# facebookresearch/robust_cvd

Hardware: AMD Instinct MI355X
Metric: GN/LM iterations/sec (and ms/iter) on 300-frame 384x224 video, 1/2/4/8 GPU (higher is better)
Workload: dtype f64

## Files before the change

### include/cvd_hip_debug.h

```cpp
#ifndef CVD_HIP_DEBUG_H
#define CVD_HIP_DEBUG_H

#include "cvd_hip.h"

#ifdef __cplusplus
extern "C" {
#endif

typedef struct cvd_debug_options {
  uint64_t struct_size;
  int32_t force_iterations;
  int32_t force_sharded_path;
  int32_t pcg_lockstep;
  int32_t stall_fused_tail_once;
} cvd_debug_options;
void cvd_debug_options_default(cvd_debug_options* o);
int32_t cvd_set_debug_options(cvd_handle* h, const cvd_debug_options* o);

int32_t cvd_set_generic_kernels(cvd_handle* h, int32_t enabled);

int32_t cvd_comm_init_local_group(cvd_handle* h, int32_t rank, int32_t world, uint64_t group_key);
int32_t cvd_comm_init_phantom(cvd_handle* h, int32_t rank, int32_t world);

int32_t cvd_block_inverse_debug(cvd_handle* h, int32_t num_blocks, int32_t block_size, const double* a, int32_t variant,
                                float* inverse, int32_t* failed);

int32_t cvd_epipolar_debug(cvd_handle* h, int32_t num_pairs, const int64_t* offsets, const float* loc, double pixel_scale,
                           double threshold_px, int32_t iterations, uint64_t seed, uint8_t* is_static_out,
                           double* fundamental_out, int32_t* best_out, int32_t* counts_out, double* hypotheses_out);
int32_t cvd_flow_masks_debug(cvd_handle* h, int32_t num_frames, int32_t height, int32_t width, int32_t channels,
                             const float* color, int32_t num_pairs, const int32_t* pair_frames, const float* flow_ab,
                             const float* flow_ba, float flow_thresh, float color_thresh, uint8_t* mask_ab, uint8_t* mask_ba,
                             int32_t* kept, float* errors, double* kernel_ms, int32_t pixels_per_thread);
int32_t cvd_dense_inverse_debug(cvd_handle* h, int32_t n, const double* a, double* inverse, int32_t* failed);
int32_t cvd_coarse_debug(cvd_handle* h, int32_t* num_unknowns, double* a_c, double* a_c_inverse, int32_t* failed);
int32_t cvd_temporal_debug(cvd_handle* h, int32_t* dims6, double* a_t, double* a_t_inverse, double* lam, int32_t* failed);
int32_t cvd_product_launch_debug(cvd_handle* h, int32_t* out6);

#ifdef __cplusplus
}
#endif
#endif
```

### robust_cvd_amd/api.py

```python
import ctypes as C
import os
import sys

from . import build as _build
from .binding import Binding
from .ctypes_types import OptParams, SolveSummary, XformDesc

_lib = None
_variant = None


class SolverOptions(C.Structure):
    _fields_ = [
        ("struct_size", C.c_uint64),
        ("pcg_relative_tolerance", C.c_double),
        ("pcg_max_iterations", C.c_int32),
        ("verbose", C.c_int32),
        ("coarse_level", C.c_int32),
        ("robust_loss", C.c_int32),
        ("dense_matrix_free", C.c_int32),
        ("block_inverse_variant", C.c_int32),
        ("coarse_dense_max_unknowns", C.c_int32),
        ("coarse_rebuild_excess", C.c_int32),
        ("coarse_update_budget", C.c_int64),
# ... 316 lines not shown
        if not os.path.exists(path):
            raise ImportError(
                f"{path} is missing: build it with `python -c 'import __graft_entry__ as g; g.build()'` "
                "(hipcc --offload-arch=gfx950). robust_cvd_amd has no CPU fallback.")
        lib = C.CDLL(path)
        lib.cvd_create.restype = C.c_void_p
        lib.cvd_create.argtypes = [C.c_int32]
        lib.cvd_last_error.restype = C.c_char_p
        lib.cvd_last_error.argtypes = [C.c_void_p]
        lib.cvd_num_active_constraints.restype = C.c_int64
        lib.cvd_abi_revision.restype = C.c_int32
        if lib.cvd_abi_revision() != ABI_REVISION:
            raise ImportError(f"{path} was built with ABI revision {lib.cvd_abi_revision()}, this binding is written against "
                              f"{ABI_REVISION} (include/cvd_hip.h: CVD_ABI_REVISION): rebuild the library")
        _lib = lib
        _variant = variant
    return _lib


def loaded_variant():
    return _variant


EXPORTED_SYMBOLS = [
    "cvd_create", "cvd_destroy", "cvd_last_error", "cvd_abi_sizes", "cvd_opt_params_default",
    "cvd_solver_options_default", "cvd_set_solver_options", "cvd_debug_options_default", "cvd_set_debug_options", "cvd_set_generic_kernels", "cvd_comm_unique_id", "cvd_comm_init", "cvd_comm_init_local_group", "cvd_comm_init_phantom", "cvd_set_pair_graph", "cvd_set_video", "cvd_set_depth", "cvd_set_depth_all",
    "cvd_set_pair_constraints", "cvd_set_pair_flows", "cvd_dense_mode_supported", "cvd_set_triplet_constraints", "cvd_set_poses", "cvd_get_poses",
    "cvd_reset_poses", "cvd_reset_depth_xforms", "cvd_reset_spatial_xforms", "cvd_grid_xform_split",
    "cvd_get_xform_desc", "cvd_num_xform_params", "cvd_get_xform_params", "cvd_set_xform_params",
    "cvd_get_pose_params", "cvd_set_pose_params", "cvd_block_size", "cvd_normalize_depth", "cvd_pose_optimization",
    "cvd_pose_optimization_step", "cvd_evaluate", "cvd_sample_pair_constraints", "cvd_get_sampled_constraints", "cvd_sample_triplet_constraints", "cvd_get_sampled_triplet_constraints", "cvd_set_dynamic_masks", "cvd_corner_min_eigenval", "cvd_dynamic_distance", "cvd_apply_depth_xforms", "cvd_depth_param_maps", "cvd_spatial_warp_maps", "cvd_flow_guided_filter", "cvd_bilateral_filter", "cvd_epipolar_static_flags", "cvd_compute_tracks", "cvd_get_tracks", "cvd_flow_consistency_masks", "cvd_consistency_loss", "cvd_consistency_loss_device", "cvd_scene_flow_loss", "cvd_scene_flow_loss_device", "cvd_spatial_losses", "cvd_spatial_losses_device", "cvd_param_chunk", "cvd_parameter_l1", "cvd_parameter_l1_device", "cvd_param_step", "cvd_param_step_device", "cvd_dataset_create", "cvd_dataset_clear", "cvd_dataset_set_colors", "cvd_dataset_set_flows", "cvd_dataset_set_depth_orig", "cvd_dataset_set_cameras", "cvd_dataset_set_xforms", "cvd_dataset_set_maps", "cvd_dataset_batch", "cvd_dataset_batch_device", "cvd_dataset_bad_indices", "cvd_get_summary", "cvd_num_records", "cvd_get_records",
    "cvd_get_kernel_times", "cvd_get_comm_times", "cvd_get_dense_times", "cvd_set_kernel_timing", "cvd_num_active_constraints", "cvd_coarse_debug", "cvd_temporal_debug", "cvd_path_info", "cvd_abi_revision",
    "cvd_block_inverse_debug", "cvd_dense_inverse_debug", "cvd_epipolar_debug", "cvd_flow_masks_debug",
    "cvd_product_launch_debug",
]

KERNEL_CLASSES = ["evaluate_assemble", "matvec_pairs", "matvec_finish", "cg_update", "block_inverse", "cost"]


class Solver(Binding):
    def __init__(self, device=0):
        lib = load_library()
        handle = lib.cvd_create(C.c_int32(device))
        if not handle:
            raise RuntimeError("cvd_create failed: " + (lib.cvd_last_error(None) or b"").decode())
        super().__init__(lib, "cvd_", handle)
        self._options = None
        self._debug = None

    def set_options(self, pcg_relative_tolerance=None, pcg_max_iterations=None, verbose=None,
                    coarse_level=None, robust_loss=None, **variants):
        debug = {k: variants.pop(k) for k in list(variants) if k in dict(DebugOptions._fields_) and k != "struct_size"}
        if debug:
            d = self._debug
            if d is None:
                d = DebugOptions()
                self._lib.cvd_debug_options_default(C.byref(d))
                self._debug = d
            for k, v in debug.items():
                setattr(d, k, int(v))
            self._check(self._fn("set_debug_options")(self._h, C.byref(d)))
        o = self._options
        if o is None:
            o = SolverOptions()
            self._lib.cvd_solver_options_default(C.byref(o))
            self._options = o
        if pcg_relative_tolerance is not None:
# ... 430 lines not shown
                                                    out.ctypes.data_as(C.POINTER(C.c_double)), C.byref(fl)))
        return out, fl.value

    def temporal_debug(self):
        import numpy as np
        dims = (C.c_int32 * 6)()
        self._check(self._fn("temporal_debug")(self._h, dims, None, None, None, None))
        if dims[0] == 0:
            return None
        n = dims[0]
        a = np.zeros((n, n))
        ai = np.zeros((n, n))
        lam = np.zeros(self.num_frames * self.block_size())
        fl = C.c_int32(0)
        dp = lambda x: x.ctypes.data_as(C.POINTER(C.c_double))
        self._check(self._fn("temporal_debug")(self._h, dims, dp(a), dp(ai), dp(lam), C.byref(fl)))
        return {"NT": n, "S": dims[1], "nn": dims[2], "step": dims[3], "Sx": dims[4], "Sy": dims[5], "a_t": a, "a_t_inverse": ai,
                "lam": lam, "failed": fl.value}

    def path_info(self):
        out = (C.c_int32 * 8)()
        self._check(self._fn("path_info")(self._h, out))
        form = {-1: "none", 0: "exact sparse factor", 1: "exact dense inverse", 2: "temporal pose level"}[out[1]]
        return {"pose_graph_level": form, "depth_grid_level": bool(out[2]), "fused_tail": bool(out[3]), "tail_disabled": bool(out[4]),
                "taps": out[5], "work_items": out[6], "cross_blocks": bool(out[7])}

    def product_launch_debug(self):
        out = (C.c_int32 * 6)()
        self._check(self._fn("product_launch_debug")(self._h, out))
        kind = {-1: "none", 0: "generic list", 1: "fast list", 2: "fast dense", 3: "cross blocks"}[out[3]]
        return {"threads": out[0], "spec": out[1], "kd": out[2], "kind": out[3], "kind_name": kind, "work_items": out[4],
                "num_cu": out[5]}

    def coarse_debug(self):
        import numpy as np
        n = C.c_int32(0)
        self._check(self._fn("coarse_debug")(self._h, C.byref(n), None, None, None))
        if n.value == 0:
            return None
        a = np.zeros((n.value, n.value))
        ai = np.zeros((n.value, n.value))
        fl = C.c_int32(0)
        self._check(self._fn("coarse_debug")(self._h, C.byref(n), a.ctypes.data_as(C.POINTER(C.c_double)),
                                             ai.ctypes.data_as(C.POINTER(C.c_double)), C.byref(fl)))
        return {"a_c": a, "a_c_inverse": ai, "failed": fl.value}
```

### robust_cvd_amd/csrc/cvd_api.hip

```cpp
#include "cvd_host.h"
#include "cvd_coarse.h"

namespace cvd {

static void poseOptimizationStep(cvd_handle* h, const cvd_opt_params& p, double depthDeformReg) {
  solve(h, p, depthDeformReg, PK_POSE_STEP);
  paramsToPoses(h, p);
}

static void poseOptimization(cvd_handle* h, const cvd_opt_params& p) {
  posesToParams(h);
  h->records.clear();
  int ctfRows = p.ctf_long, ctfCols = p.ctf_short;
  int dsoRows = p.dso_long, dsoCols = p.dso_short;
  if (h->aspect >= 1.f) {
    std::swap(ctfCols, ctfRows);
    std::swap(dsoCols, dsoRows);
  }
  int initGrid[3] = {1, 1, 1};
  if (h->ddesc.depth_type == CVD_DEPTH_GRID)
    for (int i = 0; i < 3; ++i) initGrid[i] = h->ddesc.grid_size[i];
  const int Nval = (h->ddesc.depth_type == CVD_DEPTH_IDENTITY) ? 0 : valueNumParams(h->ddesc.value_xform);
  size_t nDmax = static_cast<size_t>(h->nD());
  if (p.coarse_to_fine && h->ddesc.depth_type != CVD_DEPTH_IDENTITY && p.num_steps > 1)
// ... 889 lines not shown
  CVD_TRY(h, {
    auto& T = h->temporal;
    hipStream_t s = h->stream;
    const bool on = T.on && T.built;
    const int dims[6] = {on ? T.NT : 0, T.S, T.nn, T.step, T.Sx, T.Sy};
    for (int i = 0; i < 6; ++i) dims6[i] = dims[i];
    if (on) {
      const size_t n2 = static_cast<size_t>(T.NT) * T.NT;
      if (a_t) T.A.download(a_t, n2, s);
      if (a_t_inverse) T.Ainv.download(a_t_inverse, n2, s);
      if (lam) h->dLam.download(lam, static_cast<size_t>(h->F) * h->Bsz(), s);
      int fl = 0;
      T.fail.download(&fl, 1, s);
      HIP_CHECK(hipStreamSynchronize(s));
      if (failed) *failed = fl;
    }
  });
}
int32_t cvd_path_info(cvd_handle* h, int32_t* out8) {
  CVD_TRY(h, {
    out8[0] = h->coarseOn ? 1 : 0;
    out8[1] = !h->coarseOn ? -1 : (h->coarse.temporalPose ? 2 : (h->coarse.denseMode ? 1 : 0));
    out8[2] = h->temporal.on ? 1 : 0;
    out8[3] = h->lastFusedTail ? 1 : 0;
    out8[4] = h->tailDisabled ? 1 : 0;
    out8[5] = h->lastKD;
    out8[6] = static_cast<int32_t>(h->itemFa.size());
    out8[7] = h->lastCross ? 1 : 0;
  });
}
int32_t cvd_product_launch_debug(cvd_handle* h, int32_t* out6) {
  CVD_TRY(h, {
    for (int i = 0; i < 6; ++i) out6[i] = h->lastProduct[i];
  });
}
int32_t cvd_coarse_debug(cvd_handle* h, int32_t* num_unknowns, double* a_c, double* a_c_inverse, int32_t* failed) {
  CVD_TRY(h, {
    auto& C = h->coarse;
    if (!C.valid || !h->coarseOn) {
      *num_unknowns = 0;
    } else if (C.temporalPose) {
      const size_t n = static_cast<size_t>(C.ptN);
      *num_unknowns = static_cast<int32_t>(n);
      hipStream_t s = h->stream;
      int fl = 0;
      C.fail.download(&fl, 1, s);
      if (a_c) C.ptMat.download(a_c, n * n, s);
      if (a_c_inverse) C.ptInv.download(a_c_inverse, n * n, s);
      HIP_CHECK(hipStreamSynchronize(s));
      if (failed) *failed = fl;
    } else {
      const int F = h->F;
      const size_t n = static_cast<size_t>(F) * kCB;
      *num_unknowns = static_cast<int32_t>(n);
      hipStream_t s = h->stream;
      int fl = 0;
      C.fail.download(&fl, 1, s);
      if (a_c_inverse) {
        std::vector<double> save(n), unit(n, 0.0);
        C.rc.download(save.data(), n, s);
        HIP_CHECK(hipStreamSynchronize(s));
        DevBuf<double> scalTmp;
        scalTmp.ensure(S_COUNT);
        HIP_CHECK(hipMemsetAsync(scalTmp.p, 0, S_COUNT * sizeof(double), s));
        for (size_t k = 0; k < n; ++k) {
          unit[k] = 1.0;
// ... 47 lines not shown
```

### robust_cvd_amd/csrc/cvd_assembly.h

```cpp
#pragma once

#include "cvd_kernels.h"

namespace cvd {

template <int KD, int KS>
inline __global__ __launch_bounds__(256) void k_assemble(Layout L, Table T, const double* __restrict__ x,
                                                  const FrameConst* __restrict__ fc, const double* __restrict__ mask,
                                                  const float* __restrict__ median,
                                                  const unsigned char* __restrict__ inRange,
                                                  const unsigned char* __restrict__ rangeFlags,
                                                  const int* __restrict__ fpOff, const int* __restrict__ fpList,
                                                  double* __restrict__ gOut, double* __restrict__ hOut,
                                                  double* __restrict__ costFrame, double* __restrict__ focalG,
                                                  double* __restrict__ focalH, AsmPanels panels, int panelCap) {
  extern __shared__ __attribute__((aligned(16))) double sm[];
  const int B = L.B;
  double* Hs = sm;
  double* gs = Hs + panelCap;
  double* xf = gs + B;
  double* xo = xf + B;
  FrameConst* fcs = reinterpret_cast<FrameConst*>(xo + B);
  double* red = reinterpret_cast<double*>(fcs + 2);
  const int f = blockIdx.x;
// ... 210 lines not shown
inline __global__ __launch_bounds__(256) void k_shared_focal_fixup(Layout L, const double* __restrict__ focalG,
                                                            const double* __restrict__ focalH,
                                                            const double* __restrict__ mask, double* __restrict__ g,
                                                            double* __restrict__ hBlocks) {
  __shared__ double red[8];
  double a = 0.0, b = 0.0;
  for (int f = threadIdx.x; f < L.F; f += 256) { a += focalG[f]; b += focalH[f]; }
  a = waveSum(a);
  b = waveSum(b);
  if ((threadIdx.x & 63) == 0) { red[threadIdx.x >> 6] = a; red[4 + (threadIdx.x >> 6)] = b; }
  __syncthreads();
  if (threadIdx.x == 0) {
    const double m = mask[6];
    g[6] += (red[0] + red[1] + red[2] + red[3]) * m;
    hBlocks[static_cast<size_t>(6) * L.B + 6] += (red[4] + red[5] + red[6] + red[7]) * m * m;
  }
}

inline __global__ void k_extract_diag(Layout L, const double* __restrict__ hBlocks, double* __restrict__ out) {
  const size_t n = static_cast<size_t>(L.F) * L.B;
  const size_t i = static_cast<size_t>(blockIdx.x) * blockDim.x + threadIdx.x;
  if (i >= n) return;
  const size_t f = i / L.B, c = i - f * L.B;
  out[i] = hBlocks[(f * L.B + c) * L.B + c];
}


#ifdef CVD_ASM_PROFILE
__device__ unsigned long long g_asmProf[2048 * 16];
#define ASM_STAMP(slot) do { if (lane == 0) g_asmProf[(blockIdx.x & 2047) * 16 + (slot)] = wall_clock64(); } while (0)
#else
#define ASM_STAMP(slot) do {} while (0)
#endif
template <int KD, bool DENSE = false, bool STAGE = false, bool FOLD = false>
inline __global__ __launch_bounds__(kAsmThreads) void k_assemble_fast(Layout L, Table T, const double* __restrict__ x,
                                                       const FrameConst* __restrict__ fc,
                                                       const double* __restrict__ mask, const float* __restrict__ median,
                                                       const unsigned char* __restrict__ regOwner,
                                                       const unsigned char* __restrict__ rangeFlags,
                                                       AsmWork work,
                                                       double* __restrict__ gOut, double* __restrict__ hOut,
                                                       double* __restrict__ costFrame, double* __restrict__ focalG,
                                                       double* __restrict__ focalH, DenseRecords dr = DenseRecords{}) {
  extern __shared__ __attribute__((aligned(16))) double sm[];
  constexpr double eps = 1e-6;
  const int B = L.B;
  const int npk = B * (B + 1) / 2;
  double* Hs = sm;
  double* gs = Hs + npk;
  double* xf = gs + B;
  double* red = xf + B;
  double* xstage = red + 4 * 36;
  const AsmPart me = FOLD ? AsmPart{static_cast<int>(blockIdx.x), 0, 0, 0, 1, 0} : work.parts[blockIdx.x];
  const int f = me.frame;
  const int tid = threadIdx.x;
  constexpr int NT = kAsmThreads;
  const int wv = __builtin_amdgcn_readfirstlane(tid >> 6);
  const int lane = tid & 63;
  if (tid == 0) ASM_STAMP(0);
  for (int i = tid; i < npk; i += NT) Hs[i] = 0.0;
  if (tid < 48) red[tid] = 0.0;
  for (int i = tid; i < B; i += NT) {
    gs[i] = 0.0;
    xf[i] = x[static_cast<size_t>(f) * B + i];
  }
  __syncthreads();
  if (tid == 0) ASM_STAMP(1);

  double PP[28], gp[7];
  double GD[19];
#pragma unroll
  for (int i = 0; i < 19; ++i) GD[i] = 0.0;
  double cost = 0.0;
  double shG = 0.0, shH = 0.0;
#pragma unroll
  for (int i = 0; i < 28; ++i) PP[i] = 0.0;
#pragma unroll
  for (int i = 0; i < 7; ++i) gp[i] = 0.0;
  const int N = L.N;
  const double A = L.aspect;

  if constexpr (FOLD) {
    if (L.includeStatic) {
      const int G = L.nD;
      const int recN = dwRecordDoubles(G);
      const int e0 = dr.fpOff[f], e1 = dr.fpOff[f + 1];
      const int nOut = 36 + 13 * G;
      for (int o = tid; o < nOut; o += NT) {
        int off0, off1, c = -1, v = 0;
        if (o < 28) {
          int i = 0;
          while ((i + 1) * (i + 2) / 2 <= o) ++i;
          const int j = o - i * (i + 1) / 2;
          off0 = i * 16 + j;
          off1 = (7 + i) * 16 + 7 + j;
        } else if (o < 35) {
          off0 = (o - 28) * 16 + 14;
          off1 = (7 + o - 28) * 16 + 14;
        } else if (o == 35) {
          off0 = 256 + 40 * G;
          off1 = -1;
        } else {
          const int e = o - 36;
          c = e / G;
          v = e - c * G;
          if (c < 7) { off0 = 256 + c * G + v; off1 = 256 + 15 * G + (7 + c) * G + v; }
          else if (c == 7) { off0 = 256 + 14 * G + v; off1 = 256 + 29 * G + v; }
          else { off0 = 256 + 30 * G + (c - 8) * G + v; off1 = 256 + 35 * G + (c - 8) * G + v; }
        }
        double s = 0.0;
        for (int e = e0; e < e1; ++e) {
          const int code = dr.fpList[e];
          const int off = (code & 1) ? off1 : off0;
          if (off < 0) continue;
          for (int q = dr.recOff[code >> 1]; q < dr.recOff[(code >> 1) + 1]; ++q) s += dr.records[static_cast<size_t>(q) * recN + off];
        }
        if (o < 36) atomicAdd(&red[o], s);
        else if (c < 7) Hs[packedIdx(7 + v, c)] = s;
        else if (c == 7) gs[7 + v] = s;
        else {
          const int d = c - 8;
          const int v2 = v + (d == 0 ? 0 : (d == 1 ? 1 : L.gx + d - 3));
          if (v2 < G) atomicAdd(&Hs[packedIdx(7 + v2, 7 + v)], s);
        }
      }
    }
  } else
  if (L.includeStatic) {
    for (int u = me.u0 + wv; u < me.u1; u += NT / 64) {
      const int2 unit = work.units[u];
      const int code = __builtin_amdgcn_readfirstlane(unit.x);
      const int p = code >> 1;
      const int side = code & 1;
      const int o = side ? T.pairA[p] : T.pairB[p];
      const double* __restrict__ xo = x + static_cast<size_t>(o) * B;
      const FrameConst& Fa = side ? fc[o] : fc[f];
      const FrameConst& Fb = side ? fc[f] : fc[o];
      double* xw = xstage + wv * B;
      if constexpr (STAGE) {
        for (int i = lane; i < B; i += 64) xw[i] = xo[i];
        asm volatile("s_waitcnt vmcnt(0) lgkmcnt(0)" ::: "memory");
      }
      const double* xa = STAGE ? (side ? xw : xf) : (side ? xo : xf);
      const double* xb = STAGE ? (side ? xf : xw) : (side ? xf : xo);
      const double fya = Fa.fy, fxa = Fa.fy * A;
      const double fyb = Fb.fy;
      const double ifyb = 1.0 / fyb, ifxb = 1.0 / (fyb * A);
      const long long cBegin = T.pairOff[p] + __builtin_amdgcn_readfirstlane(unit.y);
      constexpr int kUnit = DENSE ? kAsmUnitDense : kAsmUnit;
      const long long cEnd = cBegin + kUnit < T.pairOff[p + 1] ? cBegin + kUnit : T.pairOff[p + 1];
      const int fsrc = side ? o : f, ftgt = side ? f : o;
      const long long cFirst = DENSE ? cBegin + static_cast<long long>(lane) * kDenseRun : cBegin + lane;
      const long long cStop = DENSE ? (cFirst + kDenseRun < cEnd ? cFirst + kDenseRun : cEnd) : cEnd;
      constexpr long long cStep = DENSE ? 1 : 64;
      RecordStream<true> rs;
      const int iFirst = static_cast<int>(cFirst - cBegin), iStop = static_cast<int>(cStop - cBegin);
      if constexpr (DENSE) rs.prime(T, cBegin, iFirst, iStop);
      for (long long c = cFirst; c < cStop; c += cStep) {
        float4 nd;
        float2 d;
        if constexpr (DENSE) {
          if (!rs.take(T, cBegin, static_cast<int>(c - cBegin), 1, iStop, T.pairOff[p], fsrc, ftgt, nd, d)) continue;
        } else {
          if (!loadConstraint<false>(T, c, T.pairOff[p], fsrc, ftgt, nd, d)) continue;
        }
        const double da = static_cast<double>(d.x), db = static_cast<double>(d.y);
        FastTaps<KD> ta, tb;
        fastGather<KD>(L, nd.x, nd.y, ta);
        fastGather<KD>(L, nd.z, nd.w, tb);
        double Da, Db;
        if (N == 0) {
// ... 234 lines not shown
#pragma unroll
        for (int i = 0; i < 19; ++i) GD[i] = waveSum(GD[i]);
        if (lane == 0) {
          for (int a = 0; a < N; ++a) {
            const int ct = 7 + a;
            for (int i = 0; i < 7; ++i) atomicAdd(&Hs[ct * (ct + 1) / 2 + i], GD[a * 7 + i]);
            atomicAdd(&gs[ct], GD[17 + a]);
          }
          atomicAdd(&Hs[packedIdx(7, 7)], GD[14]);
          if (N == 2) { atomicAdd(&Hs[packedIdx(8, 7)], GD[15]); atomicAdd(&Hs[packedIdx(8, 8)], GD[16]); }
        }
      }
    }
    if (lane == 0) {
#pragma unroll
      for (int i = 0; i < 28; ++i) atomicAdd(&red[i], PP[i]);
#pragma unroll
      for (int i = 0; i < 7; ++i) atomicAdd(&red[28 + i], gp[i]);
      atomicAdd(&red[35], cost);
    }
  }
  __syncthreads();
  if (tid < 28) {
    int i = 0;
    while ((i + 1) * (i + 2) / 2 <= tid) ++i;
    const int j = tid - i * (i + 1) / 2;
    Hs[packedIdx(i, j)] += red[tid];
  } else if (tid < 35) {
    gs[tid - 28] += red[tid];
  }
  __syncthreads();
  const double staticCost = 0.5 * red[35];
  __syncthreads();
  if (tid == 0) ASM_STAMP(13);
  if (L.intrOpt == kIntrShared) {
    shG = waveSum(shG);
    shH = waveSum(shH);
    if (lane == 0) { red[wv] = shG; red[16 + wv] = shH; }
    __syncthreads();
    if (tid == 0) {
      double sg = 0.0, sh = 0.0;
      for (int w = 0; w < NT / 64; ++w) { sg += red[w]; sh += red[16 + w]; }
      focalG[f] = sg;
      focalH[f] = sh;
      red[42] = sg;
      red[43] = sh;
      gs[6] = 0.0;
      Hs[packedIdx(6, 6)] = 0.0;
    }
    if (f != 0) {
      for (int j = tid; j < B; j += NT)
        if (j != 6) Hs[j > 6 ? packedIdx(j, 6) : packedIdx(6, j)] = 0.0;
    }
    __syncthreads();
  }

  if (tid == 0) ASM_STAMP(14);
  double regCost = 0.0;
  if (regOwner[f] && me.part == 0) {
    const int nr = numRegResiduals<KD>(L);
    for (int i = tid; i < nr; i += NT) {
      double r;
      int n;
      int cols[2 * KD + 2];
      double jac[2 * KD + 2];
      regResidual<KD>(L, f, i, xf, median[f], r, n, cols, jac);
      regCost += r * r;
      for (int a = 0; a < n; ++a) {
        atomicAdd(&gs[cols[a]], jac[a] * r);
        for (int b = 0; b <= a; ++b) {
          const int hi = cols[a] > cols[b] ? cols[a] : cols[b];
          const int lo = cols[a] > cols[b] ? cols[b] : cols[a];
          atomicAdd(&Hs[packedIdx(hi, lo)], jac[a] * jac[b]);
        }
      }
    }
  }
  if (tid == 0 && L.positionRegSqrt > 0.0 && me.part == 0) {
    double o3[3] = {0, 0, 0}, dg = 0.0, cst = 0.0;
    posRegFrame(L, rangeFlags, f, x, nullptr, o3, dg, cst);
    for (int i = 0; i < 3; ++i) {
      atomicAdd(&gs[i], o3[i]);
      atomicAdd(&Hs[packedIdx(i, i)], dg);
    }
    regCost += cst;
  }
  regCost = waveSum(regCost);
  __syncthreads();
  if (tid == 0) ASM_STAMP(15);
  if (lane == 0) red[wv] = regCost;
  __syncthreads();
// ... 55 lines not shown
```

### robust_cvd_amd/csrc/cvd_eval.hip

```cpp
#include "cvd_host.h"
#include "cvd_cost.h"
#include "cvd_assembly.h"
#include "cvd_triplets.h"
#include "cvd_dense_walk.h"

namespace cvd {

void launchFrameConsts(Ctx& c, const double* x) {
  launchFrameConsts(c.L, x, c.h->dFc.p, c.h->stream);
  HIP_CHECK(hipGetLastError());
}

void spinStream(hipStream_t s) {
  hipError_t e;
  while ((e = hipStreamQuery(s)) == hipErrorNotReady) {}
  HIP_CHECK(e);
}
void spinEvent(hipEvent_t ev) {
  hipError_t e;
  while ((e = hipEventQuery(ev)) == hipErrorNotReady) {}
  HIP_CHECK(e);
}
void readScalars(Ctx& c) {
  HIP_CHECK(hipMemcpyAsync(c.h->hScal, c.h->dScal.p, S_COUNT * sizeof(double), hipMemcpyDeviceToHost, c.h->stream));
// ... 94 lines not shown
  (void)x;
  cvd_handle* h = c.h;
  const size_t B = c.L.B, G = c.L.nD;
  h->dXBlocks.ensure(h->xFa.size() * B * B);
  const unsigned nP = static_cast<unsigned>(h->xFa.size());
  if (nP == 0) return;
  hipLaunchKernelGGL(k_dense_fold_cross, dim3(nP), dim3(256), 0, h->stream, c.L, crossPairs(h), h->dXDir.p, h->dDwRecOff.p,
                     h->dDwRecords.p, h->dXBlocks.p);
  int panelW = static_cast<int>(((kMaxLds - 4096) / 8) / G);
  panelW = std::max(1, std::min<int>(panelW, static_cast<int>(G)));
  const int nPanels = static_cast<int>((G + panelW - 1) / panelW);
  panelW = static_cast<int>((G + nPanels - 1) / nPanels);
  const size_t ldsGrid = static_cast<size_t>(panelW) * G * 8;
  allowLds((k_dense_gg<4>), ldsGrid);
  const int slot = h->tBegin(KC_DENSE_GG);
  for (int dir = 0; dir < 2; ++dir)
    hipLaunchKernelGGL((k_dense_gg<4>), dim3(nP, nPanels), dim3(kGgThreads), ldsGrid, h->stream, c.L, c.T, crossPairs(h), h->dXDir.p,
                       h->dDwGg.p, panelW, dir, h->dXBlocks.p);
  h->tEnd(slot);
  HIP_CHECK(hipGetLastError());
}

double evalFull(Ctx& c, const double* x, bool withStats, bool noReadBack) {
  cvd_handle* h = c.h;
  hipStream_t s = h->stream;
  launchFrameConsts(c, x);
  const size_t B = c.L.B;
  const int slot = h->tBegin(KC_ASSEMBLE);
  const bool fast = !h->forceGeneric && c.KS == 0 && fastLoss(c.L);
  const size_t ldsFast = (B * (B + 1) / 2 + 2 * B + 4 * 36) * 8;
  const size_t ldsRest = 3 * B * 8 + 2 * sizeof(FrameConst) + 4 * 36 * 8;
  int panelCap = 0;
  const bool fastFits = ldsFast <= kMaxLds;
  if (fast && fastFits) {
    h->dAsmScratch.ensure(static_cast<size_t>(h->nAsmSlots) * (B * (B + 1) / 2 + B + 4));
    const AsmWork work{h->dAsmParts.p, h->dAsmUnits.p, h->dAsmScratch.p, h->dAsmCount.p};
    const size_t ldsStage = ldsFast + static_cast<size_t>(kAsmThreads / 64) * B * 8;
    const bool stage = ldsStage <= kMaxLds;
#define CVD_LAUNCH_ASM(DENSEV, STAGEV)                                                                                     \
    CVD_DISPATCH_KD(c.KD, {                                                                                              \
      allowLds((k_assemble_fast<KD, DENSEV, STAGEV>), STAGEV ? ldsStage : ldsFast);                                        \
      hipLaunchKernelGGL((k_assemble_fast<KD, DENSEV, STAGEV>), dim3(h->nAsmParts), dim3(kAsmThreads), STAGEV ? ldsStage : ldsFast, s, \
                         c.L, c.T, x, h->dFc.p, h->dMask.p, h->dMedian.p, h->dRegOwner.p, h->dInRange.p, work, h->dG.p, h->dH.p,  \
                         h->dCostFrame.p, h->dFocal.p, h->dFocal.p + c.L.F);                                             \
    })
#ifndef CVD_ASM_STAGE
#define CVD_ASM_STAGE 1
#endif
    if (c.cross) {
      launchDenseWalk(c, x);
      if (c.KD == 1) {
        allowLds((k_assemble_fast<1, true, false, true>), ldsFast);
        hipLaunchKernelGGL((k_assemble_fast<1, true, false, true>), dim3(c.L.F), dim3(kAsmThreads), ldsFast, s, c.L, c.T, x, h->dFc.p,
                           h->dMask.p, h->dMedian.p, h->dRegOwner.p, h->dInRange.p, work, h->dG.p, h->dH.p, h->dCostFrame.p,
                           h->dFocal.p, h->dFocal.p + c.L.F, denseRecords(h));
      } else {
        allowLds((k_assemble_fast<4, true, false, true>), ldsFast);
        hipLaunchKernelGGL((k_assemble_fast<4, true, false, true>), dim3(c.L.F), dim3(kAsmThreads), ldsFast, s, c.L, c.T, x, h->dFc.p,
                           h->dMask.p, h->dMedian.p, h->dRegOwner.p, h->dInRange.p, work, h->dG.p, h->dH.p, h->dCostFrame.p,
                           h->dFocal.p, h->dFocal.p + c.L.F, denseRecords(h));
      }
    } else if (h->dense) { if (stage && CVD_ASM_STAGE) CVD_LAUNCH_ASM(true, true); else CVD_LAUNCH_ASM(true, false); }
    else { if (stage && CVD_ASM_STAGE) CVD_LAUNCH_ASM(false, true); else CVD_LAUNCH_ASM(false, false); }
#undef CVD_LAUNCH_ASM
  } else {
    if (h->dense && c.L.includeStatic) throw std::logic_error("dense mode: the generic assembly has no images to read (DenseListScope should have taken this solve)");
    const AsmPanels panels = makePanels(static_cast<int>(B), (kMaxLds - ldsRest) / 8, panelCap);
    const size_t lds = static_cast<size_t>(panelCap) * 8 + ldsRest;
    CVD_DISPATCH(c.KD, c.KS, {
      allowLds(k_assemble<KD, KS>, lds);
      hipLaunchKernelGGL((k_assemble<KD, KS>), dim3(c.L.F), dim3(256), lds, s, c.L, c.T, x, h->dFc.p, h->dMask.p,
                         h->dMedian.p, h->dRegOwner.p, h->dInRange.p, h->dFpOff.p, h->dFpList.p, h->dG.p, h->dH.p, h->dCostFrame.p,
                       h->dFocal.p, h->dFocal.p + c.L.F, panels, panelCap);
    });
  }
  HIP_CHECK(hipGetLastError());
  if (c.trip && c.TT.nGroups > 0) {
    int panelCapT = 0;
    const AsmPanels panelsT = makePanels(static_cast<int>(B), (kMaxLds - B * 8 - 256) / 8, panelCapT);
    const size_t ldsT = (static_cast<size_t>(panelCapT) + B) * 8;
    CVD_DISPATCH(c.KD, c.KS, {
      allowLds(k_assemble_triplets<KD, KS>, ldsT);
      hipLaunchKernelGGL((k_assemble_triplets<KD, KS>), dim3(c.L.F), dim3(256), ldsT, s, c.L, c.TT, x, h->dFc.p,
                         h->dMask.p, h->dFtOff.p, h->dFtList.p, h->dG.p, h->dH.p, h->dFocal.p, h->dFocal.p + c.L.F,
                         panelsT, panelCapT);
      hipLaunchKernelGGL((k_cost_triplets<KD, KS>), dim3(c.TT.nGroups), dim3(256), 0, s, c.L, c.TT, x, h->dFc.p,
                         h->dCostFrame.p);
    });
    HIP_CHECK(hipGetLastError());
  }
  if (c.L.intrOpt == CVD_INTR_SHARED) {
    hipLaunchKernelGGL(k_shared_focal_fixup, dim3(1), dim3(256), 0, s, c.L, h->dFocal.p, h->dFocal.p + c.L.F, h->dMask.p,
                       h->dG.p, h->dH.p);
    HIP_CHECK(hipGetLastError());
  }
  if (c.cross) launchCrossAssemble(c, x);
  h->tEnd(slot);
  if (h->dist()) {
    const int ct = h->tBegin(KC_COMM_EVAL);
    const size_t chunkH = static_cast<size_t>(h->ownChunk()) * B * B;
    commGroupStart(h);
// ... 40 lines not shown
```

### robust_cvd_amd/csrc/cvd_host.h

```cpp
#pragma once

#include <hip/hip_runtime.h>
#include <hip/hip_ext.h>
#include <rccl/rccl.h>
#include <rocblas/rocblas.h>
#include <rocsolver/rocsolver.h>

#include <algorithm>
#include <array>
#include <atomic>
#include <chrono>
#include <condition_variable>
#include <cmath>
#include <cstdarg>
#include <cstdint>
#include <cstdio>
#include <cstdlib>
#include <cstring>
#include <functional>
#include <limits>
#include <map>
#include <memory>
#include <mutex>
#include <set>
// ... 293 lines not shown
    DevBuf<unsigned char> elV;
    DevBuf<double> Cf, E, part, A, Ainv, sq, rT, t, tl, dotPart, rec;
    DevBuf<double> invPanel;
    DevBuf<unsigned int> invBarrier;
    DevBuf<TlStep> stepDev;
    hipEvent_t evIn = nullptr, evDone = nullptr;
    bool sidePending = false;
    double* sqPtr = nullptr;
  } temporal;
  hipEvent_t evRebuild[2] = {nullptr, nullptr};
  bool rebuildTimed = false;
  double coarseRebuildMs = 0.0, pcgIterMs = 0.0;
  std::vector<std::pair<int, int>> globalEdges;
  bool haveGlobalEdges = false;
  DevBuf<double> dRegJac;
  DevBuf<unsigned short> dRegCol;
  DevBuf<unsigned char> dRegCnt;
  RegCache regCache{};
  DevBuf<FrameConst> dFc;
  DevBuf<int> dFail;
  DevBuf<unsigned long long> dCount;
  double* hScal = nullptr;
  double* hStage[2] = {nullptr, nullptr};
  size_t hStageN[2] = {0, 0};
  double* hPcg = nullptr;
  hipEvent_t pcgEvent[2] = {nullptr, nullptr};

  cvd_solve_summary summary{};
  std::vector<cvd_iteration_record> records;

  bool lastFusedTail = false, lastCross = false;
  int lastKD = 0;
  int lastProduct[6] = {0, 0, 0, -1, 0, 0};
  bool tailDisabled = false;
  bool forceGeneric = false;

  int timing = 0;
  int timingStride = 1;
  long long timingCounter = 0;
  long long timingCounterKc[16] = {0};
  std::vector<std::pair<hipEvent_t, hipEvent_t>> evPool;
  std::vector<int> evClass;
  std::vector<int> evIter;
  int curPcgIter = -1;
  size_t evUsed = 0;
  double kcMs[KC_TOTAL] = {0};
  long long kcN[KC_TOTAL] = {0};

  ~cvd_handle_t() {
    for (auto& e : evPool) { (void)hipEventDestroy(e.first); (void)hipEventDestroy(e.second); }
    if (rbMain) (void)rocblas_destroy_handle(rbMain);
    if (comm) (void)ncclCommDestroy(comm);
    if (localGroup) leaveLocalGroup(*localGroup);
    if (hScal) (void)hipHostFree(hScal);
    for (auto& p : hStage) if (p) (void)hipHostFree(p);
    if (hPcg) (void)hipHostFree(hPcg);
    for (auto& e : pcgEvent) if (e) (void)hipEventDestroy(e);
    for (auto& e : evRebuild) if (e) (void)hipEventDestroy(e);
    if (temporal.evIn) (void)hipEventDestroy(temporal.evIn);
    if (temporal.evDone) (void)hipEventDestroy(temporal.evDone);
    if (evCoarseIn) (void)hipEventDestroy(evCoarseIn);
    if (evCoarseDone) (void)hipEventDestroy(evCoarseDone);
    if (evInvIn) (void)hipEventDestroy(evInvIn);
    if (evInvDone) (void)hipEventDestroy(evInvDone);
    if (stream3) (void)hipStreamDestroy(stream3);
    if (stream2) (void)hipStreamDestroy(stream2);
// ... 319 lines not shown
```

Measured before the change: 321.8.

## Add loss-specialised list-mode assembly walk for single-camera static disparity

Adds a templated SPEC variant of the fast assembly kernel, used when there is a single camera with static reprojection-disparity loss and non-shared intrinsics. The residual and Jacobian walk is specialised by robust-loss kind, with uniform hoisted rotations and fast reciprocals. The local-to-axis-angle rotation and the regulariser accumulation are moved into dedicated helpers. The aim is to cut per-constraint branching and generic overhead in Gauss-Newton assembly. It also adds a debug query reporting the chosen assembly launch and per-frame cost, and it duplicates a lot of numerics, which risks divergence from the generic path.

```diff
diff --git a/include/cvd_hip_debug.h b/include/cvd_hip_debug.h
--- a/include/cvd_hip_debug.h
+++ b/include/cvd_hip_debug.h
@@ -36,6 +36,7 @@
 int32_t cvd_coarse_debug(cvd_handle* h, int32_t* num_unknowns, double* a_c, double* a_c_inverse, int32_t* failed);
 int32_t cvd_temporal_debug(cvd_handle* h, int32_t* dims6, double* a_t, double* a_t_inverse, double* lam, int32_t* failed);
 int32_t cvd_product_launch_debug(cvd_handle* h, int32_t* out6);
+int32_t cvd_assembly_launch_debug(cvd_handle* h, int32_t* out6, double* cost_frame);
 
 #ifdef __cplusplus
 }
diff --git a/robust_cvd_amd/api.py b/robust_cvd_amd/api.py
--- a/robust_cvd_amd/api.py
+++ b/robust_cvd_amd/api.py
@@ -372,7 +372,7 @@
     "cvd_pose_optimization_step", "cvd_evaluate", "cvd_sample_pair_constraints", "cvd_get_sampled_constraints", "cvd_sample_triplet_constraints", "cvd_get_sampled_triplet_constraints", "cvd_set_dynamic_masks", "cvd_corner_min_eigenval", "cvd_dynamic_distance", "cvd_apply_depth_xforms", "cvd_depth_param_maps", "cvd_spatial_warp_maps", "cvd_flow_guided_filter", "cvd_bilateral_filter", "cvd_epipolar_static_flags", "cvd_compute_tracks", "cvd_get_tracks", "cvd_flow_consistency_masks", "cvd_consistency_loss", "cvd_consistency_loss_device", "cvd_scene_flow_loss", "cvd_scene_flow_loss_device", "cvd_spatial_losses", "cvd_spatial_losses_device", "cvd_param_chunk", "cvd_parameter_l1", "cvd_parameter_l1_device", "cvd_param_step", "cvd_param_step_device", "cvd_dataset_create", "cvd_dataset_clear", "cvd_dataset_set_colors", "cvd_dataset_set_flows", "cvd_dataset_set_depth_orig", "cvd_dataset_set_cameras", "cvd_dataset_set_xforms", "cvd_dataset_set_maps", "cvd_dataset_batch", "cvd_dataset_batch_device", "cvd_dataset_bad_indices", "cvd_get_summary", "cvd_num_records", "cvd_get_records",
     "cvd_get_kernel_times", "cvd_get_comm_times", "cvd_get_dense_times", "cvd_set_kernel_timing", "cvd_num_active_constraints", "cvd_coarse_debug", "cvd_temporal_debug", "cvd_path_info", "cvd_abi_revision",
     "cvd_block_inverse_debug", "cvd_dense_inverse_debug", "cvd_epipolar_debug", "cvd_flow_masks_debug",
-    "cvd_product_launch_debug",
+    "cvd_product_launch_debug", "cvd_assembly_launch_debug",
 ]
 
 KERNEL_CLASSES = ["evaluate_assemble", "matvec_pairs", "matvec_finish", "cg_update", "block_inverse", "cost"]
@@ -869,6 +869,15 @@
         return {"threads": out[0], "spec": out[1], "kd": out[2], "kind": out[3], "kind_name": kind, "work_items": out[4],
                 "num_cu": out[5]}
 
+    def assembly_launch_debug(self):
+        import numpy as np
+        out = (C.c_int32 * 6)()
+        cost = np.zeros(self.num_frames, dtype=np.float64)
+        self._check(self._fn("assembly_launch_debug")(self._h, out, cost.ctypes.data_as(C.POINTER(C.c_double))))
+        kind = {-1: "none", 0: "generic", 1: "fast list", 2: "fast dense", 3: "dense fold"}[out[3]]
+        return {"threads": out[0], "spec": out[1], "kd": out[2], "kind": out[3], "kind_name": kind, "workgroups": out[4],
+                "split_parts": out[5], "cost_frame": cost}
+
     def coarse_debug(self):
         import numpy as np
         n = C.c_int32(0)
diff --git a/robust_cvd_amd/csrc/cvd_api.hip b/robust_cvd_amd/csrc/cvd_api.hip
--- a/robust_cvd_amd/csrc/cvd_api.hip
+++ b/robust_cvd_amd/csrc/cvd_api.hip
@@ -945,6 +945,16 @@
 int32_t cvd_product_launch_debug(cvd_handle* h, int32_t* out6) {
   CVD_TRY(h, {
     for (int i = 0; i < 6; ++i) out6[i] = h->lastProduct[i];
+  });
+}
+int32_t cvd_assembly_launch_debug(cvd_handle* h, int32_t* out6, double* cost_frame) {
+  CVD_TRY(h, {
+    for (int i = 0; i < 6; ++i) out6[i] = h->lastAssembly[i];
+    const size_t F = static_cast<size_t>(h->F);
+    if (cost_frame && h->lastAssembly[3] >= 0 && h->dCostFrame.n >= F) {
+      h->dCostFrame.download(cost_frame, F, h->stream);
+      HIP_CHECK(hipStreamSynchronize(h->stream));
+    }
   });
 }
 int32_t cvd_coarse_debug(cvd_handle* h, int32_t* num_unknowns, double* a_c, double* a_c_inverse, int32_t* failed) {
diff --git a/robust_cvd_amd/csrc/cvd_assembly.h b/robust_cvd_amd/csrc/cvd_assembly.h
--- a/robust_cvd_amd/csrc/cvd_assembly.h
+++ b/robust_cvd_amd/csrc/cvd_assembly.h
@@ -266,7 +266,257 @@
 #else
 #define ASM_STAMP(slot) do {} while (0)
 #endif
-template <int KD, bool DENSE = false, bool STAGE = false, bool FOLD = false>
+
+template <int KD, int SPEC>
+__device__ __forceinline__ void asmWalkSpec(const Layout& L, const Table& T, RecordStream<false>& rs, long long cBegin, int n,
+                                            int lane, const bool side, const FrameConst& Fa, const FrameConst& Fb,
+                                            const double* __restrict__ xa, const double* __restrict__ xb, double* Hs,
+                                            double* gs, double (&PP)[28], double (&gp)[7], double (&GD)[19], double& cost) {
+  constexpr double eps = 1e-6;
+  const double A = L.aspect;
+  double RaU[9], RbU[9], dTU[3];
+#pragma unroll
+  for (int i = 0; i < 9; ++i) { RaU[i] = uniformValue(Fa.R[i]); RbU[i] = uniformValue(Fb.R[i]); }
+#pragma unroll
+  for (int i = 0; i < 3; ++i) dTU[i] = uniformValue(Fa.t[i] - Fb.t[i]);
+  const double fya = uniformValue(Fa.fy), fxa = fya * A;
+  const double fyb = uniformValue(Fb.fy);
+  const double ifyb = uniformValue(1.0 / fyb), ifxb = uniformValue(1.0 / (fyb * A));
+  for (int ci = lane; ci < n; ci += 64) {
+    float4 nd;
+    float2 d;
+    if (!rs.take(T, cBegin, ci, 64, n, 0, 0, 0, nd, d)) continue;
+    const double da = static_cast<double>(d.x), db = static_cast<double>(d.y);
+    FastTaps<KD> ta, tb;
+    fastGather<KD>(L, nd.x, nd.y, ta);
+    fastGather<KD>(L, nd.z, nd.w, tb);
+    double Da = 0.0, Db = 0.0;
+#pragma unroll
+    for (int k = 0; k < KD; ++k) {
+      if (ta.ok(k)) Da += xa[7 + ta.I(k)] * ta.Wt(k);
+      if (tb.ok(k)) Db += xb[7 + tb.I(k)] * tb.Wt(k);
+    }
+    Da *= da;
+    Db *= db;
+    const double pax = static_cast<double>(nd.x), pay = static_cast<double>(nd.y);
+    const double pbx = static_cast<double>(nd.z), pby = static_cast<double>(nd.w);
+    const double ca[3] = {pax * fxa, pay * fya, -1.0};
+    const double Rca[3] = {dot3(RaU, ca), dot3(RaU + 3, ca), dot3(RaU + 6, ca)};
+    const double v[3] = {dTU[0] + Rca[0] * Da, dTU[1] + Rca[1] * Da, dTU[2] + Rca[2] * Da};
+    const double q0 = RbU[0] * v[0] + RbU[3] * v[1] + RbU[6] * v[2];
+    const double q1 = RbU[1] * v[0] + RbU[4] * v[1] + RbU[7] * v[2];
+    const double q2 = RbU[2] * v[0] + RbU[5] * v[1] + RbU[8] * v[2];
+    const double zz = -q2;
+    const double iz = rcpFast(zz);
+    const double u = q0 * iz * ifxb;
+    const double vv = q1 * iz * ifyb;
+    double r[3];
+    r[0] = (u - pbx) * L.ws;
+    r[1] = (vv - pby) * L.ws;
+    const bool zo = !(zz < eps), bo = !(Db < eps);
+    const double izc = zo ? iz : 1.0 / eps, ibc = rcpFast(bo ? Db : eps);
+    r[2] = (izc - ibc) * L.wd;
+    const double dr2dA = zo ? (-L.wd * izc * izc) : 0.0;
+    const double dr2dDb = bo ? (L.wd * ibc * ibc) : 0.0;
+    const double sq = r[0] * r[0] + r[1] * r[1] + r[2] * r[2];
+    double w;
+    if constexpr (SPEC == 1) {
+      const double sum = 1.0 + sq * L.cauchyC;
+      w = rcpFast(sum);
+      if (!side) cost += L.cauchyB * log(sum);
+    } else {
+      const bool outer = sq > L.cauchyB;
+      const double irt = rsqrtFast(outer ? sq : 1.0);
+      w = outer ? fmax(2.2250738585072014e-308, L.robustA * irt) : 1.0;
+      if (!side) cost += outer ? (2.0 * L.robustA * (sq * irt) - L.cauchyB) : sq;
+    }
+
+    const double wiz = L.ws * iz;
+    const double m00 = wiz * ifxb, m11 = wiz * ifyb, m02 = wiz * u, m12 = wiz * vv, m22 = -dr2dA;
+    double G[3][3];
+#pragma unroll
+    for (int i = 0; i < 3; ++i) {
+      G[0][i] = m00 * RbU[i * 3 + 0] + m02 * RbU[i * 3 + 2];
+      G[1][i] = m11 * RbU[i * 3 + 1] + m12 * RbU[i * 3 + 2];
+      G[2][i] = m22 * RbU[i * 3 + 2];
+    }
+    double Jp[3][7];
+    double JD[3];
+    if (!side) {
+      const double X[3] = {Da * Rca[0], Da * Rca[1], Da * Rca[2]};
+      const double cf0 = pax * A, cf1 = pay;
+      const double dXdf[3] = {Da * (RaU[0] * cf0 + RaU[1] * cf1), Da * (RaU[3] * cf0 + RaU[4] * cf1),
+                              Da * (RaU[6] * cf0 + RaU[7] * cf1)};
+#pragma unroll
+      for (int rr = 0; rr < 3; ++rr) {
+        Jp[rr][0] = G[rr][0]; Jp[rr][1] = G[rr][1]; Jp[rr][2] = G[rr][2];
+        Jp[rr][3] = X[1] * G[rr][2] - X[2] * G[rr][1];
+        Jp[rr][4] = X[2] * G[rr][0] - X[0] * G[rr][2];
+        Jp[rr][5] = X[0] * G[rr][1] - X[1] * G[rr][0];
+        Jp[rr][6] = dot3(G[rr], dXdf);
+        JD[rr] = dot3(G[rr], Rca);
+      }
+    } else {
+#pragma unroll
+      for (int rr = 0; rr < 3; ++rr) {
+        Jp[rr][0] = -G[rr][0]; Jp[rr][1] = -G[rr][1]; Jp[rr][2] = -G[rr][2];
+        Jp[rr][3] = G[rr][1] * v[2] - G[rr][2] * v[1];
+        Jp[rr][4] = G[rr][2] * v[0] - G[rr][0] * v[2];
+        Jp[rr][5] = G[rr][0] * v[1] - G[rr][1] * v[0];
+      }
+      Jp[0][6] = -L.ws * u * ifyb;
+      Jp[1][6] = -L.ws * vv * ifyb;
+      Jp[2][6] = 0.0;
+      JD[0] = 0.0; JD[1] = 0.0; JD[2] = dr2dDb;
+    }
+    int qi = 0;
+#pragma unroll
+    for (int i = 0; i < 7; ++i) {
+      gp[i] += w * (Jp[0][i] * r[0] + Jp[1][i] * r[1] + Jp[2][i] * r[2]);
+#pragma unroll
+      for (int j = 0; j <= i; ++j) {
+        PP[qi] += w * (Jp[0][i] * Jp[0][j] + Jp[1][i] * Jp[1][j] + Jp[2][i] * Jp[2][j]);
+        ++qi;
+      }
+    }
+    double v7[7];
+#pragma unroll
+    for (int i = 0; i < 7; ++i) v7[i] = w * (Jp[0][i] * JD[0] + Jp[1][i] * JD[1] + Jp[2][i] * JD[2]);
+    const double sDD = w * (JD[0] * JD[0] + JD[1] * JD[1] + JD[2] * JD[2]);
+    const double sDr = w * (JD[0] * r[0] + JD[1] * r[1] + JD[2] * r[2]);
+    const FastTaps<KD>& tm = side ? tb : ta;
+    const double dm = side ? db : da;
+    if constexpr (KD == 1) {
+      const double fac = tm.Wt(0) * dm;
+#pragma unroll
+      for (int i = 0; i < 7; ++i) GD[i] += v7[i] * fac;
+      GD[17] += sDr * fac;
+      GD[14] += sDD * fac * fac;
+    } else {
+#pragma unroll
+      for (int ka = 0; ka < KD; ++ka) {
+        if (!tm.ok(ka)) continue;
+        const double fa = tm.Wt(ka) * dm;
+        const int ct = 7 + tm.I(ka);
+        const int rowBase = ct * (ct + 1) / 2;
+        atomicAdd(&gs[ct], sDr * fa);
+#pragma unroll
+        for (int i = 0; i < 7; ++i) atomicAdd(&Hs[rowBase + i], v7[i] * fa);
+        const double sfa = sDD * fa;
+#pragma unroll
+        for (int kb = 0; kb <= ka; ++kb) {
+          if (!tm.ok(kb)) continue;
+          const int c2 = 7 + tm.I(kb);
+          const int hi = (KD == 16 || ct > c2) ? ct : c2, lo = (KD == 16 || ct > c2) ? c2 : ct;
+          atomicAdd(&Hs[packedIdx(hi, lo)], sfa * (tm.Wt(kb) * dm));
+        }
+      }
+    }
+  }
+}
+
+template <int NT>
+__device__ __forceinline__ void asmLocalToAxisAngle(const double* __restrict__ Jl, int B, int tid, double* Hs, double* gs) {
+  double J[9];
+#pragma unroll
+  for (int i = 0; i < 9; ++i) J[i] = Jl[i];
+  for (int j = tid; j < B; j += NT) {
+    if (j >= 3 && j <= 5) continue;
+    const int i0 = j < 3 ? packedIdx(3, j) : packedIdx(j, 3);
+    const int i1 = j < 3 ? packedIdx(4, j) : packedIdx(j, 4);
+    const int i2 = j < 3 ? packedIdx(5, j) : packedIdx(j, 5);
+    const double h0 = Hs[i0], h1 = Hs[i1], h2 = Hs[i2];
+    Hs[i0] = J[0] * h0 + J[1] * h1 + J[2] * h2;
+    Hs[i1] = J[3] * h0 + J[4] * h1 + J[5] * h2;
+    Hs[i2] = J[6] * h0 + J[7] * h1 + J[8] * h2;
+  }
+  if (tid == NT - 1) {
+    double S[3][3], JS[3][3];
+#pragma unroll
+    for (int a = 0; a < 3; ++a)
+#pragma unroll
+      for (int b = 0; b < 3; ++b) S[a][b] = Hs[a >= b ? packedIdx(3 + a, 3 + b) : packedIdx(3 + b, 3 + a)];
+#pragma unroll
+    for (int a = 0; a < 3; ++a)
+#pragma unroll
+      for (int b = 0; b < 3; ++b) JS[a][b] = J[a * 3] * S[0][b] + J[a * 3 + 1] * S[1][b] + J[a * 3 + 2] * S[2][b];
+#pragma unroll
+    for (int a = 0; a < 3; ++a)
+#pragma unroll
+      for (int b = 0; b <= a; ++b)
+        Hs[packedIdx(3 + a, 3 + b)] = JS[a][0] * J[b * 3] + JS[a][1] * J[b * 3 + 1] + JS[a][2] * J[b * 3 + 2];
+    const double g0 = gs[3], g1 = gs[4], g2 = gs[5];
+    gs[3] = J[0] * g0 + J[1] * g1 + J[2] * g2;
+    gs[4] = J[3] * g0 + J[4] * g1 + J[5] * g2;
+    gs[5] = J[6] * g0 + J[7] * g1 + J[8] * g2;
+  }
+}
+
+template <int KD, int NT>
+__device__ __forceinline__ double asmRegularisersSpec(const Layout& L, int f, int tid, const double* __restrict__ xf, float median,
+                                                      double* Hs, double* gs) {
+  constexpr double eps = 1e-6;
+  double regCost = 0.0;
+  if (L.scaleRegSqrt > 0.0) {
+    const int ns = L.sregX * L.sregY;
+    const bool taps = KD > 1 || L.depthType == kDepthGlobal;
+    for (int i = tid; i < ns; i += NT) {
+      const int y = i / L.sregX, x = i - y * L.sregX;
+      const float lx = __fadd_rn(-1.f, __fdiv_rn(__fmul_rn(2.f, static_cast<float>(x)), static_cast<float>(L.sregX - 1)));
+      const float ly = __fadd_rn(-1.f, __fdiv_rn(__fmul_rn(2.f, static_cast<float>(y)), static_cast<float>(L.sregY - 1)));
+      FastTaps<KD> t;
+      fastGather<KD>(L, lx, ly, t);
+      const double d = static_cast<double>(median);
+      double D = (L.depthType == kDepthIdentity) ? d : 0.0;
+#pragma unroll
+      for (int k = 0; k < KD; ++k)
+        if (taps && t.ok(k)) D += d * xf[7 + t.I(k)] * t.Wt(k);
+      const bool o = !(D < eps);
+      const double dd = o ? D : eps;
+      const double r = L.scaleRegSqrt * (1.0 / dd - 1.0);
+      const double drdD = o ? (-L.scaleRegSqrt / (dd * dd)) : 0.0;
+      regCost += r * r;
+#pragma unroll
+      for (int ka = 0; ka < KD; ++ka) {
+        if (!(taps && t.ok(ka))) continue;
+        const int ca = 7 + t.I(ka);
+        const double ja = drdD * t.Wt(ka) * d;
+        atomicAdd(&gs[ca], ja * r);
+#pragma unroll
+        for (int kb = 0; kb <= ka; ++kb) {
+          if (!t.ok(kb)) continue;
+          const int cb = 7 + t.I(kb);
+          const int hi = ca > cb ? ca : cb, lo = ca > cb ? cb : ca;
+          atomicAdd(&Hs[packedIdx(hi, lo)], ja * (drdD * t.Wt(kb) * d));
+        }
+      }
+    }
+  }
+  Layout Lr = L;
+  Lr.scaleRegSqrt = 0.0;
+  const int nr = numRegResiduals<KD>(Lr);
+  for (int i = tid; i < nr; i += NT) {
+    double r;
+    int n;
+    int cols[2 * KD + 2];
+    double jac[2 * KD + 2];
+    regResidual<KD>(Lr, f, i, xf, median, r, n, cols, jac);
+    regCost += r * r;
+    if (n >= 1) {
+      atomicAdd(&gs[cols[0]], jac[0] * r);
+      atomicAdd(&Hs[packedIdx(cols[0], cols[0])], jac[0] * jac[0]);
+    }
+    if (n >= 2) {
+      atomicAdd(&gs[cols[1]], jac[1] * r);
+      const int hi = cols[1] > cols[0] ? cols[1] : cols[0], lo = cols[1] > cols[0] ? cols[0] : cols[1];
+      atomicAdd(&Hs[packedIdx(hi, lo)], jac[1] * jac[0]);
+      atomicAdd(&Hs[packedIdx(cols[1], cols[1])], jac[1] * jac[1]);
+    }
+  }
+  return regCost;
+}
+
+template <int KD, bool DENSE = false, bool STAGE = false, bool FOLD = false, int SPEC = 0>
 inline __global__ __launch_bounds__(kAsmThreads) void k_assemble_fast(Layout L, Table T, const double* __restrict__ x,
                                                        const FrameConst* __restrict__ fc,
                                                        const double* __restrict__ mask, const float* __restrict__ median,
@@ -288,6 +538,7 @@
   const AsmPart me = FOLD ? AsmPart{static_cast<int>(blockIdx.x), 0, 0, 0, 1, 0} : work.parts[blockIdx.x];
   const int f = me.frame;
   const int tid = threadIdx.x;
+  static_assert(SPEC == 0 || (!DENSE && !FOLD), "the specialised walk is list mode only");
   constexpr int NT = kAsmThreads;
   const int wv = __builtin_amdgcn_readfirstlane(tid >> 6);
   const int lane = tid & 63;
@@ -311,7 +562,7 @@
   for (int i = 0; i < 28; ++i) PP[i] = 0.0;
 #pragma unroll
   for (int i = 0; i < 7; ++i) gp[i] = 0.0;
-  const int N = L.N;
+  const int N = SPEC ? 1 : L.N;
   const double A = L.aspect;
 
   if constexpr (FOLD) {
@@ -371,6 +622,22 @@
       const FrameConst& Fa = side ? fc[o] : fc[f];
       const FrameConst& Fb = side ? fc[f] : fc[o];
       double* xw = xstage + wv * B;
+      if constexpr (SPEC != 0) {
+        const long long pOff = T.pairOff[p];
+        const long long cb = pOff + __builtin_amdgcn_readfirstlane(unit.y);
+        const long long pEnd = T.pairOff[p + 1];
+        const int n = static_cast<int>((cb + kAsmUnit < pEnd ? cb + kAsmUnit : pEnd) - cb);
+        RecordStream<false> rs;
+        rs.prime(T, cb, lane, n);
+        if constexpr (STAGE) {
+          for (int i = lane; i < B; i += 64) xw[i] = xo[i];
+          asm volatile("s_waitcnt vmcnt(0) lgkmcnt(0)" ::: "memory");
+        }
+        const double* xov = STAGE ? xw : xo;
+        asmWalkSpec<KD, SPEC>(L, T, rs, cb, n, lane, side != 0, Fa, Fb, side ? xov : xf,
+                              side ? xf : xov, Hs, gs, PP, gp, GD, cost);
+        continue;
+      }
       if constexpr (STAGE) {
         for (int i = lane; i < B; i += 64) xw[i] = xo[i];
         asm volatile("s_waitcnt vmcnt(0) lgkmcnt(0)" ::: "memory");
@@ -671,6 +938,10 @@
   __syncthreads();
   const double staticCost = 0.5 * red[35];
   __syncthreads();
+  if constexpr (SPEC != 0) {
+    asmLocalToAxisAngle<NT>(fc[f].Jl, B, tid, Hs, gs);
+    __syncthreads();
+  }
   if (tid == 0) ASM_STAMP(13);
   if (L.intrOpt == kIntrShared) {
     shG = waveSum(shG);
@@ -696,6 +967,9 @@
 
   if (tid == 0) ASM_STAMP(14);
   double regCost = 0.0;
+  if constexpr (SPEC != 0) {
+    if (regOwner[f] && me.part == 0) regCost = asmRegularisersSpec<KD, NT>(L, f, tid, xf, median[f], Hs, gs);
+  } else
   if (regOwner[f] && me.part == 0) {
     const int nr = numRegResiduals<KD>(L);
     for (int i = tid; i < nr; i += NT) {
diff --git a/robust_cvd_amd/csrc/cvd_eval.hip b/robust_cvd_amd/csrc/cvd_eval.hip
--- a/robust_cvd_amd/csrc/cvd_eval.hip
+++ b/robust_cvd_amd/csrc/cvd_eval.hip
@@ -150,23 +150,33 @@
   const size_t ldsRest = 3 * B * 8 + 2 * sizeof(FrameConst) + 4 * 36 * 8;
   int panelCap = 0;
   const bool fastFits = ldsFast <= kMaxLds;
+  auto recordAsm = [h](int threads, int spec, int kd, int kind, int groups, int splitParts) {
+    const int v[6] = {threads, spec, kd, kind, groups, splitParts};
+    for (int i = 0; i < 6; ++i) h->lastAssembly[i] = v[i];
+  };
   if (fast && fastFits) {
     h->dAsmScratch.ensure(static_cast<size_t>(h->nAsmSlots) * (B * (B + 1) / 2 + B + 4));
     const AsmWork work{h->dAsmParts.p, h->dAsmUnits.p, h->dAsmScratch.p, h->dAsmCount.p};
+    const int spec = (!h->dense && c.L.N == 1 && c.L.lossType == CVD_STATIC_REPRO_DISPARITY && c.L.intrOpt != CVD_INTR_SHARED)
+                         ? (c.L.robustKind == 0 ? 1 : 2) : 0;
     const size_t ldsStage = ldsFast + static_cast<size_t>(kAsmThreads / 64) * B * 8;
     const bool stage = ldsStage <= kMaxLds;
-#define CVD_LAUNCH_ASM(DENSEV, STAGEV)                                                                                     \
+#define CVD_LAUNCH_ASM_S(DENSEV, STAGEV, SPECV)                                                                            \
     CVD_DISPATCH_KD(c.KD, {                                                                                              \
-      allowLds((k_assemble_fast<KD, DENSEV, STAGEV>), STAGEV ? ldsStage : ldsFast);                                        \
-      hipLaunchKernelGGL((k_assemble_fast<KD, DENSEV, STAGEV>), dim3(h->nAsmParts), dim3(kAsmThreads), STAGEV ? ldsStage : ldsFast, s, \
+      recordAsm(kAsmThreads, SPECV, KD, DENSEV ? 2 : 1, h->nAsmParts, h->nAsmSlots);                                       \
+      allowLds((k_assemble_fast<KD, DENSEV, STAGEV, false, SPECV>), STAGEV ? ldsStage : ldsFast);                          \
+      hipLaunchKernelGGL((k_assemble_fast<KD, DENSEV, STAGEV, false, SPECV>), dim3(h->nAsmParts),                          \
+                         dim3(kAsmThreads), STAGEV ? ldsStage : ldsFast, s,                                                \
                          c.L, c.T, x, h->dFc.p, h->dMask.p, h->dMedian.p, h->dRegOwner.p, h->dInRange.p, work, h->dG.p, h->dH.p,  \
                          h->dCostFrame.p, h->dFocal.p, h->dFocal.p + c.L.F);                                             \
     })
+#define CVD_LAUNCH_ASM(DENSEV, STAGEV) CVD_LAUNCH_ASM_S(DENSEV, STAGEV, 0)
 #ifndef CVD_ASM_STAGE
 #define CVD_ASM_STAGE 1
 #endif
     if (c.cross) {
       launchDenseWalk(c, x);
+      recordAsm(kAsmThreads, 0, c.KD, 3, c.L.F, 0);
       if (c.KD == 1) {
         allowLds((k_assemble_fast<1, true, false, true>), ldsFast);
         hipLaunchKernelGGL((k_assemble_fast<1, true, false, true>), dim3(c.L.F), dim3(kAsmThreads), ldsFast, s, c.L, c.T, x, h->dFc.p,
@@ -179,12 +189,16 @@
                            h->dFocal.p, h->dFocal.p + c.L.F, denseRecords(h));
       }
     } else if (h->dense) { if (stage && CVD_ASM_STAGE) CVD_LAUNCH_ASM(true, true); else CVD_LAUNCH_ASM(true, false); }
+    else if (spec == 1) { if (stage && CVD_ASM_STAGE) CVD_LAUNCH_ASM_S(false, true, 1); else CVD_LAUNCH_ASM_S(false, false, 1); }
+    else if (spec == 2) { if (stage && CVD_ASM_STAGE) CVD_LAUNCH_ASM_S(false, true, 2); else CVD_LAUNCH_ASM_S(false, false, 2); }
     else { if (stage && CVD_ASM_STAGE) CVD_LAUNCH_ASM(false, true); else CVD_LAUNCH_ASM(false, false); }
 #undef CVD_LAUNCH_ASM
+#undef CVD_LAUNCH_ASM_S
   } else {
     if (h->dense && c.L.includeStatic) throw std::logic_error("dense mode: the generic assembly has no images to read (DenseListScope should have taken this solve)");
     const AsmPanels panels = makePanels(static_cast<int>(B), (kMaxLds - ldsRest) / 8, panelCap);
     const size_t lds = static_cast<size_t>(panelCap) * 8 + ldsRest;
+    recordAsm(256, 0, c.KD, 0, c.L.F, 0);
     CVD_DISPATCH(c.KD, c.KS, {
       allowLds(k_assemble<KD, KS>, lds);
       hipLaunchKernelGGL((k_assemble<KD, KS>), dim3(c.L.F), dim3(256), lds, s, c.L, c.T, x, h->dFc.p, h->dMask.p,
diff --git a/robust_cvd_amd/csrc/cvd_host.h b/robust_cvd_amd/csrc/cvd_host.h
--- a/robust_cvd_amd/csrc/cvd_host.h
+++ b/robust_cvd_amd/csrc/cvd_host.h
@@ -349,6 +349,7 @@
   bool lastFusedTail = false, lastCross = false;
   int lastKD = 0;
   int lastProduct[6] = {0, 0, 0, -1, 0, 0};
+  int lastAssembly[6] = {0, 0, 0, -1, 0, 0};
   bool tailDisabled = false;
   bool forceGeneric = false;
 
```

After: 328.4, median of 6. 2.0% higher.
